# sabbirhossainujjal/LLMVoX

Hardware: AMD Instinct MI355X
Metric: speech tokens/sec (+ 24kHz audio samples/sec = 320 x tokens/s; p50 first-chunk latency) (higher is better)
Workload: dtype bf16

## Files before the change

llmvox_amd/csrc/ar_kernels.hip:

```cpp
#include "ar_plan.h"

#pragma clang fp contract(off)

namespace lvx {

#ifdef LVX_TIMING
constexpr int TS_BLOCKS = 1024;
__device__ uint64_t g_lvx_ts[16 * 4 * TS_BLOCKS * 4];
#define TS_DECL uint64_t ts_[2] = {0, 0}
#define TS_MARK(i) do { if (threadIdx.x == 0) ts_[i] = __builtin_amdgcn_s_memrealtime(); } while (0)
#define TS_SAVE(tag, layer, blk)                                                                    \
  do {                                                                                               \
    if (threadIdx.x == 0) {                                                                          \
      const uint64_t te_ = __builtin_amdgcn_s_memrealtime();                                         \
      const uint64_t hw_ = (uint64_t)__builtin_amdgcn_s_getreg((31 << 11) | 4) |                    \
                           ((uint64_t)__builtin_amdgcn_s_getreg((3 << 11) | 20) << 32);              \
      uint64_t* p_ = g_lvx_ts + ((size_t)(((tag) * 4 + (layer)) * TS_BLOCKS + min((int)(blk), TS_BLOCKS - 1))) * 4; \
      p_[0] = ts_[0]; p_[1] = ts_[1]; p_[2] = te_; p_[3] = hw_;                                      \
    }                                                                                                \
  } while (0)
#else
#define TS_DECL do {} while (0)
#define TS_MARK(i) do {} while (0)
#define TS_SAVE(tag, layer, blk) do {} while (0)
// ... 1023 lines not shown
  for (int i = 0; i < 3; ++i) { k[4 * i] = kp[i].x; k[4 * i + 1] = kp[i].y; k[4 * i + 2] = kp[i].z; k[4 * i + 3] = kp[i].w; }
  float s0 = 0.f, s1 = 0.f, s2 = 0.f, s3 = 0.f;
#pragma unroll
  for (int j = 0; j < 6; ++j) {
    s0 = dot2_bf16(qs.hi[j], k[j], s0);
    s1 = dot2_bf16(qs.hi[6 + j], k[6 + j], s1);
    s2 = dot2_bf16(qs.lo[j], k[j], s2);
    s3 = dot2_bf16(qs.lo[6 + j], k[6 + j], s3);
  }
  return quad_sum((s0 + s1) + (s2 + s3));
}
__device__ __forceinline__ void slot_update_bf16(float& m, float& l, f32x2_t (&o)[12], float sc, const uint4 (&vp)[3],
                                                 bool valid) {
  uint32_t v[12];
#pragma unroll
  for (int i = 0; i < 3; ++i) { v[4 * i] = vp[i].x; v[4 * i + 1] = vp[i].y; v[4 * i + 2] = vp[i].z; v[4 * i + 3] = vp[i].w; }
  if (!valid) return;
  const float mn = fmaxf(m, sc);
  const float alpha = __builtin_amdgcn_exp2f((m - mn) * 1.4426950408889634f);
  const float p = __builtin_amdgcn_exp2f((sc - mn) * 1.4426950408889634f);
  l = l * alpha + p;
  const f32x2_t a2 = f32x2_t{alpha, alpha}, p2 = f32x2_t{p, p};
#pragma unroll
  for (int j = 0; j < 12; ++j) {
    const f32x2_t vv = f32x2_t{__uint_as_float(v[j] << 16), __uint_as_float(v[j] & 0xffff0000u)};
    o[j] = __builtin_elementwise_fma(p2, vv, o[j] * a2);
  }
  m = mn;
}
__device__ __forceinline__ void slot_softmax_step_bf16(float& m, float& l, f32x2_t (&o)[12], const QSplit& qs,
                                                       const uint4 (&kp)[3], const uint4 (&vp)[3], bool valid) {
  slot_update_bf16(m, l, o, slot_score_bf16(qs, kp), vp, valid);
}

__device__ __forceinline__ float slot_fold_wave(float m, float& l, float (&o)[24]) {
  const float M = wave_max(m);
  const float f = (m == -INFINITY) ? 0.f : expf(m - M);
  l *= f;
#pragma unroll
  for (int i = 0; i < 24; ++i) o[i] *= f;
  return M;
}

__device__ __forceinline__ int l0_next_tok(const ArState& st, int jn, int loaded) {
  if (!st.text_plan) return 384;
  return (jn + 1 < st.plan_stride) ? min(max(loaded, 0), TEXT_VOCAB - 1) : -1;
}
__device__ __forceinline__ void lds_barrier() {
  asm volatile("s_waitcnt lgkmcnt(0)" ::: "memory");
  __builtin_amdgcn_s_barrier();
  asm volatile("" ::: "memory");
}

template <typename TKV, int NW, bool QKV, bool L0, bool LA = false, int RT = 1>
__device__ __forceinline__ void attn_v2_body(const ArState st, int layer, int ns_max, int direct, int selcopy,
                                             const GemvArgs* a0) {
  constexpr int TK = NW * 16;
  constexpr bool SLOT = sizeof(TKV) < 4;
  static_assert(!QKV || (NW == 4 && sizeof(TKV) == 4), "the K-split c_attn: the fp32 parity mode's 4-wave blocks");
  static_assert(!L0 || (NW == 4 && SLOT && !QKV), "the fused layer-0 form: bf16 / fp8 KV in 4-wave blocks");
  static_assert(!LA || (NW == 4 && SLOT && !QKV && !L0), "the fused layers form: bf16 / fp8 KV in 4-wave blocks");
  constexpr bool NEWKV = QKV || L0 || LA;
  constexpr bool HIST = L0 || LA;
  constexpr int QH = NEWKV ? (3 * HD + NW * 64 - 1) / (NW * 64) : 1;
  __shared__ float wm_s[NW], wl_s[NW];
  __shared__ float wo_s[NW][4][HD];
  __shared__ float qs_s[NEWKV ? HD : 1];
  __shared__ __attribute__((aligned(16))) TKV kvh_s[NEWKV ? 2 : 1][NEWKV ? HD : 1];
  __shared__ float sv_s[L0 ? 4 : 1], sv2_s[L0 ? 4 : 1];
  __shared__ int si_s[L0 ? 4 : 1];
  __shared__ float4 sst_s;
  __shared__ __attribute__((aligned(16))) bf16_t xb_s[LA ? NW : 1][LA ? D : 8];
  __shared__ float red_s[LA ? NW : 1][LA ? 3 * HD : 1];
  const int sp = blockIdx.x, head = blockIdx.y, b = blockIdx.z;
  const int tid = threadIdx.x, wave = tid >> 6, lane = tid & 63;
  TS_DECL;
  TS_MARK(0);
  int4 rold = make_int4(-1, 0, 0, 0);
  int2 rx = make_int2(0, 0);
  bool tk = false;
  float4 lgv[L0 ? VOCAB / 1024 : 1];
  int zn[L0 ? QH : 1];
  float zg[L0 ? QH : 1], zt[L0 ? QH : 1], zp[L0 ? QH : 1];
  int jnx = 0, tnext = 384;
  int4 ri0 = make_int4(-1, 0, 0, 0);
  if constexpr (L0) {
    rold = st.rowinfo[b];
    rx = st.rowx[b];
    const unsigned pend = st.selrow[b];
    const float4* lg = reinterpret_cast<const float4*>(st.logits + (size_t)b * VOCAB);
#pragma unroll
    for (int k = 0; k < VOCAB / 1024; ++k) lgv[k] = lg[k * 256 + tid];
#pragma unroll
    for (int h = 0; h < QH; ++h) {
      const int e = min(tid + NW * 64 * h, 3 * HD - 1);
      zn[h] = (e / HD) * D + head * HD + e % HD;
      zg[h] = a0->q0_g[zn[h]];
    }
    tk = pend && rold.x >= 0;
    const int p1 = min(max(tk ? rold.y + 1 : rold.y, 0), st.max_pos - 1);
    const int t1 = tk ? rx.y : rold.z;
#pragma unroll
    for (int h = 0; h < QH; ++h) {
      zt[h] = a0->q0_text[(size_t)(t1 < 0 ? 384 : t1) * (3 * D) + zn[h]];
      zp[h] = a0->q0_pos[(size_t)p1 * (3 * D) + zn[h]];
    }
    jnx = tk ? rx.x + 1 : rx.x;
    if (st.text_plan) tnext = st.text_plan[(size_t)b * st.plan_stride + min(jnx + 1, st.plan_stride - 1)];
    ri0 = make_int4(rold.x, p1, 0, 0);
    if (rold.x < 0) {
      if (head == 0) {
        if (tid == 0) {
          st.rowinfo_n[b] = rold;
          st.rowx_n[b] = make_int2(jnx, l0_next_tok(st, jnx, tnext));
        }
        if (tid < D / 4) reinterpret_cast<float4*>(st.x + (size_t)b * D)[tid] = make_float4(0.f, 0.f, 0.f, 0.f);
      }
      return;
    }
  }
  const int4 ri = L0 ? ri0 : selcopy ? st.rowinfo_n[b] : st.rowinfo[b];
  XRow<LA ? GIN_LN_Y : GIN_LN> xr;
  float4 gam[3];
  uint4 wr[RT][6];
  int2 rxn = make_int2(0, 0);
  const uint4* wsl = nullptr;
  const int rot = LA ? (b * 7) % 18 : 0;
  auto la_tile = [&](int i) { const int j = i + rot; return j >= 18 ? j - 18 : j; };
  auto la_woff = [&](int j) { return (size_t)((j / 6) * 48 + j % 6) * (D / 32) * 64; };
  if constexpr (LA) {
    rxn = st.rowx_n[b];
#pragma unroll
    for (int j = 0; j < 3; ++j) gam[j] = *reinterpret_cast<const float4*>(a0->ln_w + j * 256 + lane * 4);
    xrow_issue(*a0, b, lane, xr);
    wsl = reinterpret_cast<const uint4*>(a0->Wf) + ((size_t)head * 6 * (D / 32) + wave * 6) * 64 + lane;
#pragma unroll
    for (int i = 0; i < RT; ++i)
#pragma unroll
      for (int kk = 0; kk < 6; ++kk) wr[i][kk] = wsl[la_woff(la_tile(i)) + kk * 64];
    __builtin_amdgcn_sched_barrier(0);
  }
  float pq[QH][QKV ? 4 : 1];
  if constexpr (QKV) {
#pragma unroll
    for (int h = 0; h < QH; ++h) {
      const int e = min(tid + NW * 64 * h, 3 * HD - 1);
      const float* pp = st.qkvp + (size_t)b * (3 * D) + (e / HD) * D + head * HD + e % HD;
#pragma unroll
      for (int k = 0; k < 4; ++k) pq[h][k] = pp[(size_t)k * st.max_streams * (3 * D)];
    }
  }
  const bool cp = selcopy && sp == 0 && head == 0 && tid == 0;
  int jn = 0;
  if (cp) {
    if constexpr (LA) jn = rxn.x;
    else jn = st.rowx_n[b].x;
    st.rowinfo[b] = ri;
    st.selrow[b] = 1u;
    if (b == 0) *st.selp = 0u;
  }
  auto copy_tail = [&]() {
    if (cp) st.rowx[b] = make_int2(jn, plan_tok(st, b, jn + 1));
  };
  const int s = ri.x;
  if (s < 0) {
    copy_tail();
    if (direct == ATTN_F32_ROWS && sp == 0 && tid < HD) st.part_o[(size_t)(b * N_HEAD + head) * NSPLIT * HD + tid] = 0.f;
    return;
  }
  const int t = ri.y + 1;
  const int ns = min(ns_max, (t + ATK - 1) / ATK);
  if (sp >= ns) return;
  const int chunk = SLOT ? (((t + ns - 1) / ns + ATK - 1) / ATK) * ATK : (t + ns - 1) / ns;
  const int k0 = sp * chunk, k1 = HIST ? t - 1 : min(t, k0 + chunk);
  const size_t base = kv_at(layer, st.kv_chunks, st.max_streams, s, head, 0);
  const size_t cstride = (size_t)st.max_streams * N_HEAD * KV_CHUNK * HD;
  const TKV* __restrict__ Kg = reinterpret_cast<const TKV*>(st.kc) + base;
  const TKV* __restrict__ Vg = reinterpret_cast<const TKV*>(st.vc) + base;
  auto krow = [&](int k) { return (size_t)(k / KV_CHUNK) * cstride + (size_t)(k % KV_CHUNK) * HD; };
  const int part = tid & 3, kq = tid >> 2;
  float q[24];
// ... 49 lines not shown
      reinterpret_cast<TKV*>(which ? st.vc : st.kc)[base + krow(ri.y) + d] = hv;
    }
  };
  auto q_from_lds = [&]() {
    lds_barrier();
#pragma unroll
    for (int i = 0; i < 24; ++i) q[i] = qs_s[part * 24 + i] * 0.10206207261596575f;
  };
  auto tile = [&](int kb, const KvPiece<TKV>(&kp)[3], const KvPiece<TKV>(&vp)[3]) {
    const bool valid = kb + kq < k1;
    if constexpr (BF) {
      uint4 ku[3], vu[3];
#pragma unroll
      for (int i = 0; i < 3; ++i) { ku[i] = reinterpret_cast<const uint4&>(kp[i]); vu[i] = reinterpret_cast<const uint4&>(vp[i]); }
      slot_softmax_step_bf16(m, l, o2, qsp, ku, vu, valid);
      return;
    }
    float kf[24], vf[24];
    if constexpr (QKV) {
      KvPiece<TKV> kx[3], vx[3];
#pragma unroll
      for (int i = 0; i < 3; ++i) { kx[i] = kp[i]; vx[i] = vp[i]; }
      if (kb + TK >= k1 && min(kb + kq, k1 - 1) == t - 1) {
#pragma unroll
        for (int i = 0; i < 3; ++i) {
          kx[i].load(kvh_s[0] + part * 24 + i * 8);
          vx[i].load(kvh_s[1] + part * 24 + i * 8);
        }
      }
#pragma unroll
      for (int i = 0; i < 3; ++i) { kx[i].get(kf + 8 * i); vx[i].get(vf + 8 * i); }
    } else {
#pragma unroll
      for (int i = 0; i < 3; ++i) { kp[i].get(kf + 8 * i); vp[i].get(vf + 8 * i); }
    }
    if constexpr (SLOT) {
      slot_softmax_step(m, l, o, q, kf, vf, valid);
      return;
    }
    float sc = 0.f;
#pragma unroll
    for (int i = 0; i < 24; ++i) sc = fmaf(q[i], kf[i], sc);
    sc = quad_sum(sc);
    if (!valid) sc = -INFINITY;
    const float mn = fmaxf(m, wave_max(sc));
    if (mn == -INFINITY) return;
    const float alpha = (m == -INFINITY) ? 0.f : expf(m - mn);
    const float p = valid ? expf(sc - mn) : 0.f;
    l = l * alpha + wave_sum(part == 0 ? p : 0.f);
#pragma unroll
    for (int i = 0; i < 24; ++i) o[i] = fmaf(valid ? p : 0.f, valid ? vf[i] : 0.f, o[i] * alpha);
    m = mn;
  };
#pragma unroll
  for (int d = 0; d < 2; ++d) issue(k0 + d * TK, kpr[d], vpr[d]);
  if constexpr (QKV) {
#pragma unroll
    for (int h = 0; h < QH; ++h) {
      const int e = tid + NW * 64 * h;
      float v = 0.f;
#pragma unroll
      for (int k = 0; k < 4; ++k) v += pq[h][k];
      newkey_put(e, v, k1 == t);
    }
    q_from_lds();
  }
  if constexpr (LA) {
    {
      float4 v[3];
      xrow_sum(xr, v);
      wave_ln_regs(v, gam);
      uint2* dst = reinterpret_cast<uint2*>(xb_s[wave]);
#pragma unroll
      for (int j = 0; j < 3; ++j) dst[j * 64 + lane] = pack4_bf16(v[j]);
    }
    asm volatile("s_waitcnt lgkmcnt(0)" ::: "memory");
    __builtin_amdgcn_wave_barrier();
    uint4 xf[6];
#pragma unroll
    for (int kk = 0; kk < 6; ++kk)
      xf[kk] = *reinterpret_cast<const uint4*>(xb_s[wave] + (wave * 6 + kk) * 32 + 8 * (lane >> 4));
    f32x4_t accp = f32x4_t{0.f, 0.f, 0.f, 0.f};
#pragma unroll
    for (int i = 0; i < 18; ++i) {
      f32x4_t acc = f32x4_t{0.f, 0.f, 0.f, 0.f};
#pragma unroll
      for (int kk = 0; kk < 6; ++kk)
        acc = __builtin_amdgcn_mfma_f32_16x16x32_bf16(__builtin_bit_cast(bf16x8_t, wr[i % RT][kk]),
                                                      __builtin_bit_cast(bf16x8_t, xf[kk]), acc, 0, 0, 0);
      if (i + RT < 18) {
#pragma unroll
        for (int kk = 0; kk < 6; ++kk)
          wr[i % RT][kk] = wsl[la_woff(la_tile(i + RT)) + kk * 64];
      }
      if (i > 0 && (lane & 15) == 0) {
#pragma unroll
        for (int r = 0; r < 4; ++r) red_s[wave][la_tile(i - 1) * 16 + 4 * (lane >> 4) + r] = accp[r];
      }
      accp = acc;
      __builtin_amdgcn_sched_barrier(0);
    }
    if ((lane & 15) == 0) {
#pragma unroll
      for (int r = 0; r < 4; ++r) red_s[wave][la_tile(17) * 16 + 4 * (lane >> 4) + r] = accp[r];
    }
    lds_barrier();
#pragma unroll
    for (int h = 0; h < QH; ++h) {
      const int e = tid + NW * 64 * h;
      if (e < 3 * HD) {
        float v = 0.f;
#pragma unroll
        for (int w = 0; w < NW; ++w) v += red_s[w][e];
        newkey_put(e, v, true);
      }
    }
    q_from_lds();
    TS_MARK(1);
  }
  if constexpr (L0) {
    const GemvArgs& a = *a0;
    row_best_wave([&](int k) { return lgv[k]; }, sv_s, sv2_s, si_s);
    lds_barrier();
    int4 rn = rold;
    if (tk) {
      const Best r = row_best_merge(sv_s, sv2_s, si_s, st.logits + (size_t)b * VOCAB, lane);
      const int sl = rold.x, p = rold.y + 1, j = rx.x;
      rn = make_int4(sl, min(p, st.max_pos - 1), rx.y, min(max(r.i, 0), VOCAB - 1));
      if (head == 0 && tid == 0) {
        if (p >= st.max_pos) atomicOr(st.err, 1);
        if (j < st.plan_stride) {
          st.tok_plan[(size_t)b * st.plan_stride + j] = r.i;
          if (st.margin_plan) st.margin_plan[(size_t)b * st.plan_stride + j] = r.v - r.v2;
        }
        st.prev[sl] = r.i;
        st.pos[sl] = p;
        st.rowstep[b] = j + 1;
      }
    }
    if (head == 0 && tid == 0) {
      st.rowinfo_n[b] = rn;
      st.rowx_n[b] = make_int2(jnx, l0_next_tok(st, jnx, tnext));
    }
    float zc[QH];
#pragma unroll
    for (int h = 0; h < QH; ++h) zc[h] = a.q0_code[(size_t)min(max(rn.w, 0), VOCAB - 1) * (3 * D) + zn[h]];
    if (wave == 0) {
      const float4 s4 = q0_row_stats(a, rn, b, lane, head == 0);
      if (lane == 0) sst_s = s4;
    }
    lds_barrier();
    const float4 ss = sst_s;
#pragma unroll
    for (int h = 0; h < QH; ++h) {
      const int e = tid + NW * 64 * h;
      const float v = q0_out(ss, rn.y, zt[h], zc[h], zp[h], zg[h]);
      newkey_put(e, v, true);
    }
    q_from_lds();
    TS_MARK(1);
  }
  if constexpr (BF) qsplit_make(q, qsp);
  for (int kb = k0; kb < k1; kb += 2 * TK) {
#pragma unroll
    for (int d = 0; d < 2; ++d) {
      if (d > 0 && kb + d * TK >= k1) break;
      tile(kb + d * TK, kpr[d], vpr[d]);
      issue(kb + (d + 2) * TK, kpr[d], vpr[d]);
    }
  }
  if constexpr (HIST) {
    const bool mine = kq == (t - 1) % TK;
    KvPiece<TKV> kx[3], vx[3];
#pragma unroll
    for (int i = 0; i < 3; ++i) {
      kx[i].load(kvh_s[0] + part * 24 + i * 8);
      vx[i].load(kvh_s[1] + part * 24 + i * 8);
    }
    if constexpr (BF) {
      uint4 ku[3], vu[3];
#pragma unroll
      for (int i = 0; i < 3; ++i) { ku[i] = reinterpret_cast<const uint4&>(kx[i]); vu[i] = reinterpret_cast<const uint4&>(vx[i]); }
      slot_softmax_step_bf16(m, l, o2, qsp, ku, vu, mine);
    } else {
      float kf[24], vf[24];
#pragma unroll
      for (int i = 0; i < 3; ++i) { kx[i].get(kf + 8 * i); vx[i].get(vf + 8 * i); }
      slot_softmax_step(m, l, o, q, kf, vf, mine);
    }
    TS_SAVE(9, layer, head + N_HEAD * b);
  }
  if constexpr (BF) {
#pragma unroll
    for (int j = 0; j < 12; ++j) { o[2 * j] = o2[j].x; o[2 * j + 1] = o2[j].y; }
  }
  if constexpr (SLOT) {
    m = slot_fold_wave(m, l, o);
    l = wave_sum(part == 0 ? l : 0.f);
  }
#pragma unroll
  for (int i = 0; i < 24; ++i) {
    float v = o[i];
    v += dpp_f32<0x128>(v);
    v += dpp_f32<0x124>(v);
    o[i] = v;
  }
  if ((lane & 15) < 4) {
#pragma unroll
    for (int i = 0; i < 24; ++i) wo_s[wave][lane >> 4][(lane & 3) * 24 + i] = o[i];
  }
  TS_MARK(1);
  if (lane == 0) { wm_s[wave] = m; wl_s[wave] = l; }
  __syncthreads();
  TS_SAVE(2, layer, sp + gridDim.x * (head + N_HEAD * b));
  copy_tail();
  if (tid < HD) {
    float M = wm_s[0];
#pragma unroll
    for (int w = 1; w < NW; ++w) M = fmaxf(M, wm_s[w]);
    float ov = 0.f, lv = 0.f;
#pragma unroll
    for (int w = 0; w < NW; ++w) {
      const float f = (wm_s[w] == -INFINITY) ? 0.f : expf(wm_s[w] - M);
      ov += f * ((wo_s[w][0][tid] + wo_s[w][1][tid]) + (wo_s[w][2][tid] + wo_s[w][3][tid]));
      lv += f * wl_s[w];
    }
    if (direct == ATTN_F32_ROWS) {
      st.part_o[(size_t)(b * N_HEAD + head) * NSPLIT * HD + tid] = ov * (1.0f / lv);
      return;
    }
    if (direct) {
      st.xn[direct == ATTN_XN_PACKED ? xfrag(b, head * HD + tid, D) : (size_t)b * D + head * HD + tid] = f32_to_bf16(ov * (1.0f / lv));
      return;
    }
    st.part_o[((size_t)(b * N_HEAD + head) * NSPLIT + sp) * HD + tid] = ov;
    if (tid == 0) {
      float* ml = st.part_ml + ((size_t)(b * N_HEAD + head) * NSPLIT + sp) * 2;
      ml[0] = M;
      ml[1] = lv;
    }
  }
}

template <typename TKV, int NW, bool QKV = false>
__global__ __launch_bounds__(NW * 64) void ar_attn_v2_kernel(ArState st, int layer, int ns_max, int direct,
                                                         int selcopy) {
  attn_v2_body<TKV, NW, QKV, false>(st, layer, ns_max, direct, selcopy, nullptr);
}

template <typename TKV>
__global__ __launch_bounds__(256) LVX_LOADS_FIRST void ar_attn_l0_kernel(GemvArgs a, int direct) {
  attn_v2_body<TKV, 4, false, true>(a.st, 0, 1, direct, 0, &a);
}

#ifndef LVX_LA_RT
#define LVX_LA_RT 3
#endif
template <typename TKV>
__global__ __launch_bounds__(256) __attribute__((amdgpu_waves_per_eu(1, 2))) void ar_attn_la_kernel(GemvArgs a, int direct,
                                                                                                    int selcopy) {
  attn_v2_body<TKV, 4, false, false, true, LVX_LA_RT>(a.st, a.layer, 1, direct, selcopy, &a);
}

__device__ __forceinline__ void hist_store(const ArState& st, int s, int p, int tok) {
  if (st.rowstep && p < st.max_pos) st.hist[(size_t)s * st.max_pos + p] = (uint16_t)tok;
}

template <bool HIST = false>
__device__ __forceinline__ void argmax_row(const ArState& st, int b, int4 ri, float* sv, float* sv2, int* si) {
  const int tid = threadIdx.x, wave = tid >> 6, lane = tid & 63;
  const float4* lg = reinterpret_cast<const float4*>(st.logits + (size_t)b * VOCAB);
  row_best_wave([&](int k) { return lg[k * 256 + tid]; }, sv, sv2, si);
  __syncthreads();
  if (wave == 0) {
    const Best r = row_best_merge(sv, sv2, si, st.logits + (size_t)b * VOCAB, lane);
    if (lane == 0) {
      argmax_commit(st, b, ri, r);
      if constexpr (HIST) hist_store(st, ri.x, ri.y, r.i);
    }
  }
}

__global__ __launch_bounds__(256) void ar_argmax_kernel(ArState st) {
  __shared__ float sv[4], sv2[4];
  __shared__ int si[4];
  const int b = blockIdx.x;
  const int4 ri = st.rowinfo[b];
  if (ri.x < 0) return;
  argmax_row(st, b, ri, sv, sv2, si);
}

__device__ __forceinline__ unsigned z_key(float z) {
  const unsigned u = __float_as_uint(z);
  return u ^ ((u >> 31) ? 0xffffffffu : 0x80000000u);
}
__device__ __forceinline__ float key_z(unsigned k) {
  return __uint_as_float(k ^ ((k >> 31) ? 0x80000000u : 0xffffffffu));
}
__device__ __forceinline__ int wave_scan_i32(int v, int lane) {
  v += dpp_i32<0x111>(v);
  v += dpp_i32<0x112>(v);
  v += dpp_i32<0x114>(v);
  v += dpp_i32<0x118>(v);
  const int r0 = __builtin_amdgcn_readlane(v, 15), r1 = __builtin_amdgcn_readlane(v, 31);
  const int r2 = __builtin_amdgcn_readlane(v, 47), row = lane >> 4;
  return v + (row == 0 ? 0 : row == 1 ? r0 : row == 2 ? r0 + r1 : r0 + r1 + r2);
}
__device__ __forceinline__ void wave_scan_f32(float x, int lane, float& excl, float& total) {
  float v = x;
  v += dpp_f32<0x111>(v);
  v += dpp_f32<0x112>(v);
  v += dpp_f32<0x114>(v);
  v += dpp_f32<0x118>(v);
  const float r0 = lane_f32(v, 15), r1 = lane_f32(v, 31), r2 = lane_f32(v, 47), r3 = lane_f32(v, 63);
// ... 1354 lines not shown
  }
  const int B = p.B;
  const bool ln = p.path == PATH_MFMA_LN, mf = ln || p.path == PATH_MFMA_ROWS, fm = p.fused_mlp;
  a.xpk = p.xpk;
  set_op_operands(a, w, op, l);
  a.yacc = mf ? a.st.yacc : nullptr;
  a.yfx = fm ? a.st.yfx : nullptr;
  a.add_y = l > 0;
  switch (op) {
    case OP_QKV:
      if (!(p.sel == SEL_ARGMAX || (mf ? p.sel == SEL_EMBED || p.sel == SEL_Q0_ROWS || (ln && p.sel == SEL_LN_GRAN)
                                       : p.sel == SEL_GRAN)))
        ar_plan_bug(p, "c_attn");
      if (l == 0 && p.l0_fused) {
      } else if (l > 0 && p.la_fused) {
      } else if (l == 0 && p.sel == SEL_LN_GRAN) {
        launch_mfma_ln<OUT_QKV, MLMODE_EMBED_SELECT>(a, s);
      } else if (l == 0 && p.sel == SEL_Q0_ROWS) {
        hipLaunchKernelGGL(ar_q0_rows_kernel, dim3(3 * D / 256, B), dim3(256), 0, s, a);
      } else if (l == 0 && p.sel == SEL_EMBED) {
        hipLaunchKernelGGL(ar_embed_select_kernel<>, dim3(B), dim3(256), 0, s, a);
        launch_mfma2<768, OUT_QKV>(a, s);
      } else if (ln) {
        if (l == 0) launch_mfma_ln<OUT_QKV, MLMODE_EMBED>(a, s);
        else launch_mfma_ln<OUT_QKV, MLMODE_LN_Y>(a, s);
      } else if (mf) {
        if (l == 0) hipLaunchKernelGGL((ar_rows_kernel<RMODE_EMBED>), dim3(B), dim3(64), 0, s, a);
        else if (l == 1 && p.l0_fused) hipLaunchKernelGGL((ar_rows_kernel<RMODE_LN_Y_COPY>), dim3(B), dim3(64), 0, s, a);
        else hipLaunchKernelGGL((ar_rows_kernel<RMODE_LN_Y>), dim3(B), dim3(64), 0, s, a);
        launch_mfma2<768, OUT_QKV>(a, s);
      } else if (l == 0 && p.q0_gran) {
        hipLaunchKernelGGL(ar_q0_gran_kernel, dim3(3 * D / 256), dim3(256), 0, s, a);
      } else if (l == 0 && p.sel == SEL_GRAN) {
        launch_gemv<TW, 768, 1, 2, GIN_EMBED_SELECT, OUT_QKV>(a, s);
      } else if (l == 0) {
        launch_gemv<TW, 768, 1, 2, GIN_EMBED, OUT_QKV>(a, s);
      } else if (fm) {
        launch_gemv<TW, 768, 1, 2, GIN_LN_Y, OUT_QKV>(a, s);
      } else {
        launch_gemv<TW, 768, 1, 2, GIN_LN, OUT_QKV>(a, s);
      }
      break;
    case OP_ATTN:
      if (l == 0 && p.l0_fused) {
        if (p.kv_dtype == LVX_DTYPE_BF16)
          hipLaunchKernelGGL(ar_attn_l0_kernel<bf16_t>, dim3(1, N_HEAD, B), dim3(256), 0, s, a, p.attn_direct);
        else if (p.kv_dtype == LVX_DTYPE_FP8)
          hipLaunchKernelGGL(ar_attn_l0_kernel<fp8_t>, dim3(1, N_HEAD, B), dim3(256), 0, s, a, p.attn_direct);
        else ar_plan_bug(p, "fused layer-0 attention");
        break;
      }
      if (l > 0 && p.la_fused) {
        a.Wf = w.f_attn[l]; a.ln_w = w.ln1[l];
        if (p.kv_dtype == LVX_DTYPE_BF16)
          hipLaunchKernelGGL(ar_attn_la_kernel<bf16_t>, dim3(1, N_HEAD, B), dim3(256), 0, s, a, p.attn_direct, (int)(l == 1));
        else if (p.kv_dtype == LVX_DTYPE_FP8)
          hipLaunchKernelGGL(ar_attn_la_kernel<fp8_t>, dim3(1, N_HEAD, B), dim3(256), 0, s, a, p.attn_direct, (int)(l == 1));
        else ar_plan_bug(p, "fused layers attention");
        break;
      }
      launch_attn(a.st, p.kv_dtype, B, l, s, p.nsplit, p.attn_direct, p.selcopy && l == 0, false, p.attn8);
      break;
    case OP_CPROJ:
      if (mf) {
        if (!ln) a.add_y = p.la_fused && l > 0;
        if (p.nsplit > 1) launch_merge_bf16(a.st, B, p.nsplit, s, a.xpk);
        a.ln_w = w.ln2[l];
        if (!ln) launch_mfma2<768, OUT_RESID_STATS>(a, s, true);
        else launch_mfma2<768, OUT_RESID>(a, s);
      } else {
        launch_gemv<TW, 768, 1, 1, GIN_MERGE, OUT_RESID>(a, s);
      }
      break;
    case OP_FC:
      if (fm) {
        const bf16_t* wfc = reinterpret_cast<const bf16_t*>(w.w_fc[l]);
        const bf16_t* wpk = reinterpret_cast<const bf16_t*>(w.w_mproj_pk[l]);
        if (B <= 1) hipLaunchKernelGGL((ar_mlp_fused_kernel<1, 16>), dim3(DFF / 16), dim3(256), 0, s, a, wfc, wpk);
        else hipLaunchKernelGGL((ar_mlp_fused_kernel<2, 16>), dim3(DFF / 16), dim3(256), 0, s, a, wfc, wpk);
      } else if (ln) {
        launch_mfma_ln<OUT_GELU_BF16, MLMODE_LN>(a, s);
      } else if (mf) {
        a.gsum = w.fc_gsum[l];
        launch_mfma2<768, OUT_GELU_BF16, M2X_LN_AFTER>(a, s);
      } else {
        launch_gemv<TW, 768, 1, 2, GIN_LN, OUT_GELU>(a, s);
      }
      break;
    case OP_MPROJ:
      if (fm) return false;
      if (ln && YCS < YCOPIES)
        hipLaunchKernelGGL((ar_mfma2_kernel<DFF / YCS, 1, OUT_SPLITK, DFF>), dim3(D / 16, YCS), dim3(DFF / YCS / 192 * 64), 0, s, a);
      else if (mf) launch_mproj_split<OUT_SPLITK>(a, s);
      else launch_gemv<TW, 3072, 4, 2, GIN_H, OUT_RESID>(a, s);
      break;
    case OP_LM_HEAD:
      if (ln) {
        launch_mfma_ln<OUT_LOGITS, MLMODE_LN_Y>(a, s);
      } else if (mf) {
        hipLaunchKernelGGL((ar_rows_kernel<RMODE_LN_Y>), dim3(B), dim3(64), 0, s, a);
        launch_mfma2<768, OUT_LOGITS>(a, s);
      } else if (p.sel == SEL_GRAN) {
        if (fm) launch_gemv<TW, 768, 1, 2, GIN_LN_Y, OUT_LOGITS_GRAN>(a, s);
        else launch_gemv<TW, 768, 1, 2, GIN_LN, OUT_LOGITS_GRAN>(a, s);
      } else if (fm) {
        launch_gemv<TW, 768, 1, 2, GIN_LN_Y, OUT_LOGITS>(a, s);
      } else {
        launch_gemv<TW, 768, 1, 2, GIN_LN, OUT_LOGITS>(a, s);
      }
      break;
  }
// ... 409 lines not shown
```

llmvox_amd/csrc/ar_plan.h:

```cpp
#pragma once
#include <stdio.h>
#include <stdlib.h>

#include "lvx_internal.h"

namespace lvx {

enum { OP_QKV = 0, OP_ATTN = 1, OP_CPROJ = 2, OP_FC = 3, OP_MPROJ = 4, OP_LM_HEAD = 5 };
enum ArOut {
  OUT_QKV = 0, OUT_RESID = 1, OUT_GELU = 2, OUT_LOGITS = 3, OUT_GELU_BF16 = 5, OUT_SPLITK = 6, OUT_RESID_STATS = 7,
  OUT_LOGITS_GRAN = 9
};
enum { GIN_LN = 0, GIN_H = 1, GIN_MERGE = 2, GIN_EMBED = 3, GIN_LN_Y = 4, GIN_EMBED_SELECT = 5 };
enum { RMODE_LN = 0, RMODE_EMBED = 3, RMODE_LN_Y = 4, RMODE_LN_Y_F32 = 5, RMODE_EMBED_F32 = 6, RMODE_LN_Y_COPY = 7 };
enum { M2X_NONE = 0, M2X_LN_AFTER = 1 };
enum { MLMODE_LN = 0, MLMODE_EMBED = 3, MLMODE_LN_Y = 4, MLMODE_EMBED_SELECT = 7 };
enum { BIN_LN = 0, BIN_ROWS = 1, BIN_EMBED = 3 };
enum { FIN_LN = 0, FIN_H = 1, FIN_MERGE = 2, FIN_EMBED = 3, FIN_ATTN_ROWS = 4, FIN_LN_ROWS = 6 };
enum { ATTN_PARTIALS = 0, ATTN_XN = 1, ATTN_XN_PACKED = 2, ATTN_F32_ROWS = 3 };

enum ArPath { PATH_GEMV, PATH_MFMA_LN, PATH_MFMA_ROWS, PATH_BT, PATH_F32B };
enum ArSelect { SEL_ARGMAX = 0, SEL_GRAN = 1, SEL_EMBED = 2, SEL_LN_GRAN = 3, SEL_Q0_ROWS = 4, SEL_SAMPLE = 5 };
enum ArEndCommit { END_NONE, END_SELECT_FINAL, END_ARGMAX };

struct ArStepPlan {
  int B, kv_dtype;
  bool bf16, row;
  ArPath path;
  ArSelect sel;
  ArEndCommit end;
  int nsplit, attn_direct;
  bool attn8, selcopy;
  bool l0_fused;
  bool fused_mlp;
  bool q0_gran;
  int xpk;
  bool ksplit, qsplit;
  bool la_fused;
};

constexpr int MFMA_BATCH_MIN = 3;
constexpr int LM8_ROWS = 8;
constexpr int ATTN_BLOCKS = 256;
inline int attn_ns_max(int B) {
  int ns = NSPLIT;
  while (ns > 1 && ns * N_HEAD * B > ATTN_BLOCKS) ns >>= 1;
  return ns;
}

[[noreturn]] inline void ar_plan_bug(const ArStepPlan& p, const char* where) {
  fprintf(stderr, "llmvox: %s: no kernel for select form %d on path %d at B = %d\n", where, (int)p.sel, (int)p.path, p.B);
  abort();
}

inline ArSelect ar_plan_select(const Opts& o, const ArStepPlan& p, bool q0) {
  if (!o.defer_select) return SEL_ARGMAX;
  if (p.path == PATH_GEMV) return p.B <= 2 ? SEL_GRAN : SEL_ARGMAX;
  if (p.B < 4) return SEL_ARGMAX;
  if (p.path == PATH_BT) return SEL_EMBED;
  if (p.path == PATH_F32B) return p.qsplit ? SEL_EMBED : SEL_ARGMAX;
  if (o.l0q && q0 && p.B <= 32) return SEL_Q0_ROWS;
  if (o.defer_select == 1 && p.path == PATH_MFMA_LN && p.B <= LM8_ROWS) return SEL_LN_GRAN;
  return SEL_EMBED;
}

inline ArStepPlan ar_plan_step(const Opts& o_, int wdtype, int kvdtype, int B, bool row, bool q0, bool sample = false) {
  sample = sample && !row;
  Opts o = o_;
  if (sample) o.defer_select = 0;
  ArStepPlan p{};
  p.B = B; p.kv_dtype = kvdtype; p.bf16 = wdtype == LVX_DTYPE_BF16; p.row = row;
  const bool batched = !row && B >= MFMA_BATCH_MIN && B <= 64;
  if (!batched || (!p.bf16 && !o.f32b)) p.path = PATH_GEMV;
  else if (!p.bf16) p.path = PATH_F32B;
  else if (o.bt && (B > 32 || o.bt == 2)) p.path = PATH_BT;
  else p.path = B <= o.ln_max ? PATH_MFMA_LN : PATH_MFMA_ROWS;
  const bool mf = p.path == PATH_MFMA_LN || p.path == PATH_MFMA_ROWS;
  p.ksplit = p.path == PATH_F32B && !(o.exp & 512);
  p.qsplit = p.ksplit && B <= 32 && !(o.exp & 1024);

  p.sel = row ? SEL_ARGMAX : sample ? SEL_SAMPLE : ar_plan_select(o, p, q0);
  p.end = p.sel == SEL_ARGMAX || p.sel == SEL_SAMPLE ? END_NONE : p.sel == SEL_GRAN ? END_SELECT_FINAL : END_ARGMAX;
  p.selcopy = p.sel == SEL_GRAN || p.sel == SEL_LN_GRAN || p.sel == SEL_Q0_ROWS;
  p.q0_gran = p.sel == SEL_GRAN && o.l0q && q0;
  p.fused_mlp = p.path == PATH_GEMV && p.bf16 && o.fuse_mlp && B <= 2;

  p.attn8 = mf && B >= 5 && (B <= 8 || (kvdtype == LVX_DTYPE_FP8 && B <= 16));
  p.nsplit = p.path == PATH_GEMV ? NSPLIT : (mf && (B > 8 || p.attn8)) ? 1 : attn_ns_max(B);
  p.l0_fused = o.l0a && p.sel == SEL_Q0_ROWS && p.nsplit == 1 && !p.attn8 && B >= 9 && kvdtype != LVX_DTYPE_F32;
  p.la_fused = o.laf && p.l0_fused;
  p.xpk = (p.path == PATH_MFMA_ROWS && B <= 32) ? 1 : 0;
  p.attn_direct = p.nsplit > 1 || !(mf || p.path == PATH_F32B) ? ATTN_PARTIALS
                  : p.path == PATH_F32B ? ATTN_F32_ROWS : p.xpk ? ATTN_XN_PACKED : ATTN_XN;
  return p;
}

}
```

llmvox_amd/csrc/lvx_api.cpp:

```cpp
#include <hip/hip_runtime.h>

#include <cmath>
#include <cstdio>
#include <cstdlib>
#include <algorithm>
#include <atomic>
#include <cstring>
#include <functional>
#include <map>
#include <mutex>
#include <string>
#include <tuple>
#include <vector>

#include "llmvox.h"
#include "ar_plan.h"

using namespace lvx;

namespace lvx {
static const Opts kDefaultOpts{};
static thread_local const Opts* t_opts = nullptr;
const Opts& opts() { return t_opts ? *t_opts : kDefaultOpts; }
OptScope::OptScope(const Opts* o) : prev(t_opts) { t_opts = o; }
// ... 761 lines not shown

int lvx_stream_history(lvx_ctx* c, int slot, int pos0, int n, int32_t* tokens, int write, void* stream) {
  NEED_FINAL(c);
  if (slot < 0 || slot >= c->cfg.max_streams) return fail(LVX_E_ARG, "slot out of range");
  if (!tokens) return fail(LVX_E_ARG, "null tokens");
  if (pos0 < 0 || n < 1 || (long long)pos0 + n > (long long)c->cfg.max_positions)
    return fail(LVX_E_CAPACITY, "entries outside the slot's history");
  HIP_TRY(hipSetDevice(c->cfg.device));
  launch_history(c->st, slot, pos0, n, tokens, write != 0, (hipStream_t)stream);
  HIP_TRY(hipGetLastError());
  return LVX_OK;
}

int lvx_sample_kept(lvx_ctx* c, int B, int32_t* dst, void* stream) {
  NEED_FINAL(c);
  if (B < 1 || B > c->cfg.max_streams || !dst) return fail(LVX_E_ARG, "bad B/dst");
  HIP_TRY(hipSetDevice(c->cfg.device));
  HIP_TRY(hipMemcpyAsync(dst, c->st.smp_kept(), (size_t)B * 16, hipMemcpyDeviceToDevice, (hipStream_t)stream));
  return LVX_OK;
}

int lvx_stream_position(lvx_ctx* c, int slot, int* pos_out, void* stream) {
  NEED_FINAL(c);
  if (slot < 0 || slot >= c->cfg.max_streams || !pos_out) return fail(LVX_E_ARG, "bad slot/pos_out");
  HIP_TRY(hipSetDevice(c->cfg.device));
  int32_t v[2];
  launch_err_take(c->st.err, 1, 0, c->st.err + 3, (hipStream_t)stream);
  HIP_TRY(hipMemcpyAsync(&v[0], c->st.pos + slot, 4, hipMemcpyDeviceToHost, (hipStream_t)stream));
  HIP_TRY(hipMemcpyAsync(&v[1], c->st.err + 3, 4, hipMemcpyDeviceToHost, (hipStream_t)stream));
  HIP_TRY(hipStreamSynchronize((hipStream_t)stream));
  *pos_out = v[0];
  return bits_status(v[1]);
}

int lvx_set_option(lvx_ctx* c, const char* name, int value) {
  if (!c || !name) return fail(LVX_E_ARG, "null argument");
  std::string n(name);
  std::lock_guard<std::mutex> lk(c->mu);
  Opts& o = c->opts;
  if (n == "defer_select") o.defer_select = value;
  else if (n == "fuse_mlp") o.fuse_mlp = value != 0;
  else if (n == "bt") o.bt = std::min(std::max(value, 0), 2);
  else if (n == "codec_g2") o.codec_g2 = value != 0;
  else if (n == "codec_skinny") o.codec_skinny = value != 0;
  else if (n == "codec_g3") o.codec_g3 = value != 0;
  else if (n == "codec_g3f") o.codec_g3f = value == 1 ? 1 : 2;
  else if (n == "codec_exp") o.codec_exp = value;
  else if (n == "exp") o.exp = value;
  else if (n == "f32b") o.f32b = value != 0;
  else if (n == "ln_max") o.ln_max = std::min(std::max(value, 2), 8);
  else if (n == "l0q") o.l0q = value != 0;
  else if (n == "l0a") o.l0a = value != 0;
  else if (n == "laf") o.laf = value != 0;
  else if (n == "fmt_group") o.fmt_group = std::min(std::max(value, 0), 32);
  else return fail(LVX_E_NAME, "unknown option " + n);
  ++c->opt_epoch;
  return LVX_OK;
}

int lvx_set_capture_stream(lvx_ctx* c, void* stream) {
  if (!c) return fail(LVX_E_ARG, "null ctx");
  std::lock_guard<std::mutex> lk(c->mu);
  c->capture_stream = (hipStream_t)stream;
  return LVX_OK;
}

int lvx_set_graphs(lvx_ctx* c, int enable) {
  if (!c) return fail(LVX_E_ARG, "null ctx");
  c->use_graphs = enable != 0;
  return LVX_OK;
}

int lvx_ar_forward_row(lvx_ctx* c, int slot, int pos, const float* emb_row, float* logits, void* stream) {
  NEED_FINAL(c);
  if (slot < 0 || slot >= c->cfg.max_streams) return fail(LVX_E_ARG, "slot out of range");
  if (pos < 0 || pos >= BLOCK_SIZE)
    return fail(LVX_E_CAPACITY, "Cannot forward sequence of length " + std::to_string(pos + 1) +
                                    ", block size is only " + std::to_string(BLOCK_SIZE));
  if (pos >= c->cfg.max_positions)
    return fail(LVX_E_CAPACITY, "position " + std::to_string(pos) + " exceeds the KV capacity " +
                                    std::to_string(c->cfg.max_positions));
  if (!emb_row || !logits) return fail(LVX_E_ARG, "null emb_row/logits");
  HIP_TRY(hipSetDevice(c->cfg.device));
  const Opts o = c->opts_snapshot();
  OptScope os(&o);
  ar_launch_step(c->arw, c->st, ar_plan_step(o, c->cfg.weight_dtype, c->cfg.kv_dtype, 1, true, false), emb_row, slot,
                 pos, logits, (hipStream_t)stream);
  HIP_TRY(hipGetLastError());
  return LVX_OK;
}

static int cached_graph(lvx_ctx* c, const GraphKey& key, hipStream_t s,
                        const std::function<void(hipStream_t)>& launch, hipGraphExec_t* out) {
  const unsigned epoch = c->opt_epoch;
  if (c->graph_epoch != epoch) {
    for (auto& kv : c->graphs) (void)hipGraphExecDestroy(kv.second);
    c->graphs.clear();
    c->graph_epoch = epoch;
  }
  auto it = c->graphs.find(key);
  if (it == c->graphs.end()) {
    hipStream_t cs = c->capture_stream ? c->capture_stream : s;
    if (!cs) {
      if (!c->own_capture_stream) HIP_TRY(hipStreamCreateWithFlags(&c->own_capture_stream, hipStreamNonBlocking));
      cs = c->own_capture_stream;
    }
// ... 1010 lines not shown
```

llmvox_amd/csrc/lvx_internal.h:

```cpp
#pragma once
#include <hip/hip_runtime.h>
#include <stdint.h>
#include <string>

#include "lvx_common.h"
#include "llmvox.h"
#include "pcm_host.h"

namespace lvx {

constexpr int N_LAYER = 4, N_HEAD = 8, D = 768, HD = 96, DFF = 3072, VOCAB = 4096;
constexpr int TEXT_DIM = 256, SPEECH_DIM = 512, TEXT_VOCAB = 386, BLOCK_SIZE = 8192;
constexpr int NSPLIT = 16;
constexpr int KV_CHUNK = 64;
__host__ __device__ inline size_t kv_at(size_t layer, size_t chunks, size_t streams, int s, int head, int pos) {
  return (((((layer * chunks + (size_t)(pos / KV_CHUNK)) * streams + s) * 8 + head) * KV_CHUNK) + (size_t)(pos % KV_CHUNK)) * 96;
}
#ifndef LVX_YCOPIES
#define LVX_YCOPIES 4
#endif
constexpr int YCOPIES = LVX_YCOPIES;
constexpr int LM_MAX_BLOCKS = 1024;
struct Opts {
  int defer_select = 1;
  int fuse_mlp = 1;
  int bt = 1;
  int codec_g2 = 1, codec_skinny = 1, codec_g3 = 1, codec_g3f = 2;
  int codec_exp = 0;
  int exp = 0;
  int f32b = 1;
  int ln_max = 8;
  int l0q = 1;
  int l0a = 1;
  int laf = 1;
  int fmt_group = 0;
};
const Opts& opts();
struct OptScope {
  explicit OptScope(const Opts* o);
  ~OptScope();
  OptScope(const OptScope&) = delete;
  OptScope& operator=(const OptScope&) = delete;
  const Opts* prev;
};

struct ArWeights {
  const float* wpe = nullptr;
  const float* text_table = nullptr;
  const float* codebook = nullptr;
  const float* ln1[N_LAYER] = {};
  const float* ln2[N_LAYER] = {};
  const float* lnf = nullptr;
  const void* w_attn[N_LAYER] = {};
  const void* w_aproj[N_LAYER] = {};
  const void* w_fc[N_LAYER] = {};
  const void* w_mproj[N_LAYER] = {};
  const void* w_mproj_pk[N_LAYER] = {};
  const float* fc_gsum[N_LAYER] = {};
  const void* w_lm = nullptr;
  const float* q0_text = nullptr;
  const float* q0_code = nullptr;
  const float* q0_pos = nullptr;
  const float* q0_g = nullptr;
  const void* f_attn[N_LAYER] = {};
  const void* f_aproj[N_LAYER] = {};
  const void* f_fc[N_LAYER] = {};
  const void* f_mproj[N_LAYER] = {};
  const void* f_lm = nullptr;
};

struct ArState {
  int32_t* slots = nullptr;
  const int32_t* text_plan = nullptr;
  int32_t* rowstep = nullptr;
  int32_t* tok_plan = nullptr;
  float* margin_plan = nullptr;
  int plan_stride = 1;
  int4* rowinfo = nullptr;
  int4* rowinfo_n = nullptr;
  int2* rowx = nullptr;
  int2* rowx_n = nullptr;
  uint32_t* selp = nullptr;
  uint32_t* selrow = nullptr;
  int32_t* pos = nullptr;
  int32_t* prev = nullptr;
  uint4* smp = nullptr;
  __host__ __device__ uint4* smp_kept() const { return smp + 2 * (size_t)max_streams; }
// ... 139 lines not shown
```

Before: 255,900.

## Overlap K/V projection MFMAs with attention history tiles in fused layers kernel

In the fused layers attention kernel, only the Q-projection tiles of the c_attn GEMV are computed before attention starts. The remaining K/V projection MFMA tiles are interleaved with the first groups of KV-history tiles, and the new K/V values are reduced and written afterwards. This hides the projection weight streaming behind attention loads for batches of 17 or more. The tile order is changed to a per-batch rotation within the Q and KV groups. The cost is more register pressure and extra barriers.

```diff
diff --git a/llmvox_amd/csrc/ar_kernels.hip b/llmvox_amd/csrc/ar_kernels.hip
--- a/llmvox_amd/csrc/ar_kernels.hip
+++ b/llmvox_amd/csrc/ar_kernels.hip
@@ -1099,7 +1099,7 @@
   asm volatile("" ::: "memory");
 }
 
-template <typename TKV, int NW, bool QKV, bool L0, bool LA = false, int RT = 1>
+template <typename TKV, int NW, bool QKV, bool L0, bool LA = false, int RT = 1, int OVW = 0>
 __device__ __forceinline__ void attn_v2_body(const ArState st, int layer, int ns_max, int direct, int selcopy,
                                              const GemvArgs* a0) {
   constexpr int TK = NW * 16;
@@ -1107,6 +1107,8 @@
   static_assert(!QKV || (NW == 4 && sizeof(TKV) == 4), "the K-split c_attn: the fp32 parity mode's 4-wave blocks");
   static_assert(!L0 || (NW == 4 && SLOT && !QKV), "the fused layer-0 form: bf16 / fp8 KV in 4-wave blocks");
   static_assert(!LA || (NW == 4 && SLOT && !QKV && !L0), "the fused layers form: bf16 / fp8 KV in 4-wave blocks");
+  static_assert(OVW == 0 || (LA && 12 % OVW == 0 && (12 / OVW) % 2 == 0),
+                "the overlapped form: whole groups of k / v tiles, an even number of them (the KV register sets alternate)");
   constexpr bool NEWKV = QKV || L0 || LA;
   constexpr bool HIST = L0 || LA;
   constexpr int QH = NEWKV ? (3 * HD + NW * 64 - 1) / (NW * 64) : 1;
@@ -1173,7 +1175,10 @@
   int2 rxn = make_int2(0, 0);
   const uint4* wsl = nullptr;
   const int rot = LA ? (b * 7) % 18 : 0;
-  auto la_tile = [&](int i) { const int j = i + rot; return j >= 18 ? j - 18 : j; };
+  auto la_tile = [&](int i) {
+    if constexpr (OVW > 0) return la_tile_order(b, i);
+    const int j = i + rot; return j >= 18 ? j - 18 : j;
+  };
   auto la_woff = [&](int j) { return (size_t)((j / 6) * 48 + j % 6) * (D / 32) * 64; };
   if constexpr (LA) {
     rxn = st.rowx_n[b];
@@ -1329,6 +1334,40 @@
     for (int i = 0; i < 24; ++i) o[i] = fmaf(valid ? p : 0.f, valid ? vf[i] : 0.f, o[i] * alpha);
     m = mn;
   };
+  [[maybe_unused]] uint4 xf[LA ? 6 : 1];
+  [[maybe_unused]] f32x4_t accp = f32x4_t{0.f, 0.f, 0.f, 0.f};
+  [[maybe_unused]] auto la_wput = [&](int i) __attribute__((always_inline)) {
+    if ((lane & 15) == 0) {
+#pragma unroll
+      for (int r = 0; r < 4; ++r) red_s[wave][la_tile(i) * 16 + 4 * (lane >> 4) + r] = accp[r];
+    }
+  };
+  [[maybe_unused]] auto la_wstep = [&](int i, bool put_prev) __attribute__((always_inline)) {
+    f32x4_t acc = f32x4_t{0.f, 0.f, 0.f, 0.f};
+#pragma unroll
+    for (int kk = 0; kk < 6; ++kk)
+      acc = __builtin_amdgcn_mfma_f32_16x16x32_bf16(__builtin_bit_cast(bf16x8_t, wr[i % RT][kk]),
+                                                    __builtin_bit_cast(bf16x8_t, xf[kk]), acc, 0, 0, 0);
+    if (i + RT < 18) {
+#pragma unroll
+      for (int kk = 0; kk < 6; ++kk) wr[i % RT][kk] = wsl[la_woff(la_tile(i + RT)) + kk * 64];
+    }
+    if (put_prev) la_wput(i - 1);
+    accp = acc;
+    __builtin_amdgcn_sched_barrier(0);
+  };
+  [[maybe_unused]] auto la_wsum = [&](int lo, int hi) __attribute__((always_inline)) {
+#pragma unroll
+    for (int h = 0; h < QH; ++h) {
+      const int e = tid + NW * 64 * h;
+      if (e >= lo && e < hi) {
+        float v = 0.f;
+#pragma unroll
+        for (int w = 0; w < NW; ++w) v += red_s[w][e];
+        newkey_put(e, v, true);
+      }
+    }
+  };
 #pragma unroll
   for (int d = 0; d < 2; ++d) issue(k0 + d * TK, kpr[d], vpr[d]);
   if constexpr (QKV) {
@@ -1353,46 +1392,24 @@
     }
     asm volatile("s_waitcnt lgkmcnt(0)" ::: "memory");
     __builtin_amdgcn_wave_barrier();
-    uint4 xf[6];
 #pragma unroll
     for (int kk = 0; kk < 6; ++kk)
       xf[kk] = *reinterpret_cast<const uint4*>(xb_s[wave] + (wave * 6 + kk) * 32 + 8 * (lane >> 4));
-    f32x4_t accp = f32x4_t{0.f, 0.f, 0.f, 0.f};
-#pragma unroll
-    for (int i = 0; i < 18; ++i) {
-      f32x4_t acc = f32x4_t{0.f, 0.f, 0.f, 0.f};
-#pragma unroll
-      for (int kk = 0; kk < 6; ++kk)
-        acc = __builtin_amdgcn_mfma_f32_16x16x32_bf16(__builtin_bit_cast(bf16x8_t, wr[i % RT][kk]),
-                                                      __builtin_bit_cast(bf16x8_t, xf[kk]), acc, 0, 0, 0);
-      if (i + RT < 18) {
-#pragma unroll
-        for (int kk = 0; kk < 6; ++kk)
-          wr[i % RT][kk] = wsl[la_woff(la_tile(i + RT)) + kk * 64];
-      }
-      if (i > 0 && (lane & 15) == 0) {
-#pragma unroll
-        for (int r = 0; r < 4; ++r) red_s[wave][la_tile(i - 1) * 16 + 4 * (lane >> 4) + r] = accp[r];
-      }
-      accp = acc;
-      __builtin_amdgcn_sched_barrier(0);
-    }
-    if ((lane & 15) == 0) {
-#pragma unroll
-      for (int r = 0; r < 4; ++r) red_s[wave][la_tile(17) * 16 + 4 * (lane >> 4) + r] = accp[r];
-    }
-    lds_barrier();
-#pragma unroll
-    for (int h = 0; h < QH; ++h) {
-      const int e = tid + NW * 64 * h;
-      if (e < 3 * HD) {
-        float v = 0.f;
-#pragma unroll
-        for (int w = 0; w < NW; ++w) v += red_s[w][e];
-        newkey_put(e, v, true);
-      }
-    }
-    q_from_lds();
+    if constexpr (OVW == 0) {
+#pragma unroll
+      for (int i = 0; i < 18; ++i) la_wstep(i, i > 0);
+      la_wput(17);
+      lds_barrier();
+      la_wsum(0, 3 * HD);
+      q_from_lds();
+    } else {
+#pragma unroll
+      for (int i = 0; i < 6; ++i) la_wstep(i, i > 0);
+      la_wput(5);
+      lds_barrier();
+      la_wsum(0, HD);
+      q_from_lds();
+    }
     TS_MARK(1);
   }
   if constexpr (L0) {
@@ -1438,13 +1455,29 @@
     TS_MARK(1);
   }
   if constexpr (BF) qsplit_make(q, qsp);
-  for (int kb = k0; kb < k1; kb += 2 * TK) {
+  constexpr int OVG = OVW > 0 ? 12 / OVW : 0;
+  if constexpr (OVW > 0) {
+#pragma unroll
+    for (int g = 0; g < OVG; ++g) {
+      if (g * TK < k1) tile(g * TK, kpr[g & 1], vpr[g & 1]);
+      issue((g + 2) * TK, kpr[g & 1], vpr[g & 1]);
+#pragma unroll
+      for (int j = 0; j < OVW; ++j) la_wstep(6 + g * OVW + j, g + j > 0);
+    }
+  }
+  for (int kb = OVW > 0 ? OVG * TK : k0; kb < k1; kb += 2 * TK) {
 #pragma unroll
     for (int d = 0; d < 2; ++d) {
       if (d > 0 && kb + d * TK >= k1) break;
       tile(kb + d * TK, kpr[d], vpr[d]);
       issue(kb + (d + 2) * TK, kpr[d], vpr[d]);
     }
+  }
+  if constexpr (OVW > 0) {
+    la_wput(17);
+    lds_barrier();
+    la_wsum(HD, 3 * HD);
+    lds_barrier();
   }
   if constexpr (HIST) {
     const bool mine = kq == (t - 1) % TK;
@@ -1533,10 +1566,13 @@
 #ifndef LVX_LA_RT
 #define LVX_LA_RT 3
 #endif
-template <typename TKV>
+#ifndef LVX_LA_OVW
+#define LVX_LA_OVW 2
+#endif
+template <typename TKV, int OVW>
 __global__ __launch_bounds__(256) __attribute__((amdgpu_waves_per_eu(1, 2))) void ar_attn_la_kernel(GemvArgs a, int direct,
                                                                                                     int selcopy) {
-  attn_v2_body<TKV, 4, false, false, true, LVX_LA_RT>(a.st, a.layer, 1, direct, selcopy, &a);
+  attn_v2_body<TKV, 4, false, false, true, LVX_LA_RT, OVW>(a.st, a.layer, 1, direct, selcopy, &a);
 }
 
 __device__ __forceinline__ void hist_store(const ArState& st, int s, int p, int tok) {
@@ -2997,11 +3033,11 @@
       }
       if (l > 0 && p.la_fused) {
         a.Wf = w.f_attn[l]; a.ln_w = w.ln1[l];
-        if (p.kv_dtype == LVX_DTYPE_BF16)
-          hipLaunchKernelGGL(ar_attn_la_kernel<bf16_t>, dim3(1, N_HEAD, B), dim3(256), 0, s, a, p.attn_direct, (int)(l == 1));
-        else if (p.kv_dtype == LVX_DTYPE_FP8)
-          hipLaunchKernelGGL(ar_attn_la_kernel<fp8_t>, dim3(1, N_HEAD, B), dim3(256), 0, s, a, p.attn_direct, (int)(l == 1));
-        else ar_plan_bug(p, "fused layers attention");
+        const bool bf = p.kv_dtype == LVX_DTYPE_BF16;
+        if (!bf && p.kv_dtype != LVX_DTYPE_FP8) ar_plan_bug(p, "fused layers attention");
+        auto k = p.la_overlap ? (bf ? ar_attn_la_kernel<bf16_t, LVX_LA_OVW> : ar_attn_la_kernel<fp8_t, LVX_LA_OVW>)
+                              : (bf ? ar_attn_la_kernel<bf16_t, 0> : ar_attn_la_kernel<fp8_t, 0>);
+        hipLaunchKernelGGL(k, dim3(1, N_HEAD, B), dim3(256), 0, s, a, p.attn_direct, (int)(l == 1));
         break;
       }
       launch_attn(a.st, p.kv_dtype, B, l, s, p.nsplit, p.attn_direct, p.selcopy && l == 0, false, p.attn8);
diff --git a/llmvox_amd/csrc/ar_plan.h b/llmvox_amd/csrc/ar_plan.h
--- a/llmvox_amd/csrc/ar_plan.h
+++ b/llmvox_amd/csrc/ar_plan.h
@@ -37,7 +37,12 @@
   int xpk;
   bool ksplit, qsplit;
   bool la_fused;
+  bool la_overlap;
 };
+
+__host__ __device__ inline int la_tile_order(int b, int i) {
+  return i < 6 ? (i + 5 * b) % 6 : 6 + (i - 6 + 7 * b) % 12;
+}
 
 constexpr int MFMA_BATCH_MIN = 3;
 constexpr int LM8_ROWS = 8;
@@ -89,6 +94,7 @@
   p.nsplit = p.path == PATH_GEMV ? NSPLIT : (mf && (B > 8 || p.attn8)) ? 1 : attn_ns_max(B);
   p.l0_fused = o.l0a && p.sel == SEL_Q0_ROWS && p.nsplit == 1 && !p.attn8 && B >= 9 && kvdtype != LVX_DTYPE_F32;
   p.la_fused = o.laf && p.l0_fused;
+  p.la_overlap = o.lao && p.la_fused && B >= 17;
   p.xpk = (p.path == PATH_MFMA_ROWS && B <= 32) ? 1 : 0;
   p.attn_direct = p.nsplit > 1 || !(mf || p.path == PATH_F32B) ? ATTN_PARTIALS
                   : p.path == PATH_F32B ? ATTN_F32_ROWS : p.xpk ? ATTN_XN_PACKED : ATTN_XN;
diff --git a/llmvox_amd/csrc/lvx_api.cpp b/llmvox_amd/csrc/lvx_api.cpp
--- a/llmvox_amd/csrc/lvx_api.cpp
+++ b/llmvox_amd/csrc/lvx_api.cpp
@@ -837,6 +837,7 @@
   else if (n == "l0q") o.l0q = value != 0;
   else if (n == "l0a") o.l0a = value != 0;
   else if (n == "laf") o.laf = value != 0;
+  else if (n == "lao") o.lao = value != 0;
   else if (n == "fmt_group") o.fmt_group = std::min(std::max(value, 0), 32);
   else return fail(LVX_E_NAME, "unknown option " + n);
   ++c->opt_epoch;
diff --git a/llmvox_amd/csrc/lvx_internal.h b/llmvox_amd/csrc/lvx_internal.h
--- a/llmvox_amd/csrc/lvx_internal.h
+++ b/llmvox_amd/csrc/lvx_internal.h
@@ -33,6 +33,7 @@
   int l0q = 1;
   int l0a = 1;
   int laf = 1;
+  int lao = 1;
   int fmt_group = 0;
 };
 const Opts& opts();
```

Result: no change. 258,200 (median of 6 runs) (+0.9%).
